# jizongFox/Deep-Co-Training-for-Semi-Supervised-Image-Segmentation

Hardware: AMD Instinct MI355X
Metric: co-train imgs/sec/node (lab+unlab), 2xUNet ACDC 256x256 (higher is better)
Workload: dtype bf16; 1 GPU; cfg2: 2xUNet co-training (CE + JSD), ACDC-shaped 256x256 C=4, bs 8+8 per GPU; global_batch=8+8, parallelism=dp1, inputs=blob-structured synthetic slices (tests/helpers.py::blob_batches)

## Files before the change

deep-co-training-for-semi-supervised-image-segmentation_amd/csrc/dct_common.h:

```cpp
#pragma once
#include <hip/hip_runtime.h>
#include <cstdio>
#include <stdint.h>
#include "../../include/dct.h"

typedef __bf16 bf16_t;
typedef __attribute__((ext_vector_type(8))) __bf16 bf16x8;
typedef __attribute__((ext_vector_type(4))) __bf16 bf16x4;
typedef __attribute__((ext_vector_type(2))) __bf16 bf16x2;
typedef _Float16 f16_t;
typedef __attribute__((ext_vector_type(8))) _Float16 f16x8;
typedef __attribute__((ext_vector_type(4))) _Float16 f16x4;
typedef __attribute__((ext_vector_type(16))) float f32x16;
typedef __attribute__((ext_vector_type(4))) float f32x4;
typedef __attribute__((ext_vector_type(2))) float f32x2;

#define DCT_WAVE 64

template <typename T> struct dct_type_of;
template <> struct dct_type_of<float> { static constexpr int id = DCT_F32; };
template <> struct dct_type_of<bf16_t> { static constexpr int id = DCT_BF16; };
template <> struct dct_type_of<f16_t> { static constexpr int id = DCT_F16; };

__device__ __forceinline__ float to_f32(float v) { return v; }
// ... 65 lines not shown
  *reinterpret_cast<dct_u32x2*>(p) = __builtin_bit_cast(dct_u32x2, v);
#endif
}

__device__ __forceinline__ unsigned dct_positive_bits8(dct_u32x4 w) {
  unsigned t[4];
#pragma unroll
  for (int k = 0; k < 4; ++k)
    asm("v_pk_max_i16 %0, %1, %2\n\tv_pk_min_u16 %0, %0, %3" : "=&v"(t[k]) : "v"(w[k]), "v"(0u), "v"(0x00010001u));
  const unsigned u = t[0] | (t[1] << 2) | (t[2] << 4) | (t[3] << 6);
  return u | (u >> 15);
}

void dct_prof_begin(int cls, hipStream_t s);
void dct_prof_end(int cls, hipStream_t s);
extern int g_dct_prof_on;

extern thread_local char g_dct_last_plan[200];
#define DCT_PLAN_NOTE(...) snprintf(g_dct_last_plan, sizeof(g_dct_last_plan), __VA_ARGS__)

extern int g_dct_skip_families;
enum { DCT_DIAG_IGEMM_SPLIT_MAX_TILES = 1002, DCT_DIAG_IGEMM_SPLIT_MIN_KITERS = 1003,
       DCT_DIAG_IGEMM_POOL = 1005,
       DCT_DIAG_STEM_DGRAD_MFMA = 1008,
       DCT_DIAG_SKIP_FAMILIES = 1100 };
enum { DCT_FAM_IGEMM2 = 1, DCT_FAM_IGEMM3M = 2, DCT_FAM_IGEMM3P = 4, DCT_FAM_WGRAD2 = 8, DCT_FAM_WGRAD3 = 16, DCT_FAM_FOLDS = 32,
       DCT_FAM_ADAM = 64, DCT_FAM_POINTWISE = 128 };
#define DCT_LAUNCH_FAM(fam, cls, kernel, grid, block, shmem, stream, ...)              \
  do {                                                                                 \
    if (g_dct_skip_families & (fam)) break;                                            \
    DCT_LAUNCH(cls, kernel, grid, block, shmem, stream, __VA_ARGS__);                  \
  } while (0)

#define DCT_LAUNCH(cls, kernel, grid, block, shmem, stream, ...)                       \
  do {                                                                                 \
    if (((cls) == DCT_PROF_POINTWISE && (g_dct_skip_families & 128)) || ((cls) == DCT_PROF_ADAM && (g_dct_skip_families & 64))) break; \
    if (g_dct_prof_on) dct_prof_begin((cls), (stream));                                \
    hipLaunchKernelGGL(kernel, grid, block, shmem, stream, __VA_ARGS__);               \
    if (g_dct_prof_on) dct_prof_end((cls), (stream));                                  \
  } while (0)

static inline int dct_check_launch() {
  return hipGetLastError() == hipSuccess ? DCT_OK : DCT_ERR_LAUNCH;
}

static inline unsigned div_up(long long a, long long b) { return (unsigned)((a + b - 1) / b); }
// ... 1 lines not shown
```

deep-co-training-for-semi-supervised-image-segmentation_amd/csrc/igemm.hip:

```cpp
#include <algorithm>
#include "igemm_common.h"

extern int g_tune_lean;

namespace {


template <typename T> struct Mfma;
template <> struct Mfma<bf16_t> {
  static constexpr int KSTEP = 16;
  __device__ static __forceinline__ void run(const char* a_row, const char* b_row, int half, f32x16& acc, int kk) {
    const bf16x8 a = *reinterpret_cast<const bf16x8*>(a_row + kk * 32 + half * 16);
    const bf16x8 b = *reinterpret_cast<const bf16x8*>(b_row + kk * 32 + half * 16);
    acc = __builtin_amdgcn_mfma_f32_32x32x16_bf16(a, b, acc, 0, 0, 0);
  }
};
template <> struct Mfma<float> {
  static constexpr int KSTEP = 2;
  __device__ static __forceinline__ void run(const char* a_row, const char* b_row, int half, f32x16& acc, int kk) {
    const float a = *reinterpret_cast<const float*>(a_row + (kk * 2 + half) * 4);
    const float b = *reinterpret_cast<const float*>(b_row + (kk * 2 + half) * 4);
    acc = __builtin_amdgcn_mfma_f32_32x32x2f32(a, b, acc, 0, 0, 0);
  }
};
// ... 456 lines not shown
      *reinterpret_cast<f32x4*>(slab + (long long)row * p.N + cc * 4) = v;
    }
    return;
  }
#pragma unroll
  for (int j = 0; j < TM; ++j) {
    const int m = m0 + wm * WTM + j * 32 + l31;
    if (m >= p.M) continue;
    const int hw = p.Ho * p.Wo;
    const int n = m / hw, rem = m - n * hw;
    const int oy = rem / p.Wo, ox = rem - oy * p.Wo;
#pragma unroll
    for (int i = 0; i < TN; ++i) {
#pragma unroll
      for (int q = 0; q < 4; ++q) {
        const int c = n0 + wn * WTN + i * 32 + 8 * q + 4 * half;
        float v[4] = {acc[i][j][4 * q + 0], acc[i][j][4 * q + 1], acc[i][j][4 * q + 2], acc[i][j][4 * q + 3]};
        epilogue_store4<bf16_t>(p, n, oy, ox, c, v);
      }
    }
  }
}

template <int BN, int NWM, int NWN, int ABUFS>
__global__ __launch_bounds__(NWM * NWN * 64) void igemm3m_kernel(IgemmParams p, int tiles_x, int tiles_y) {
  constexpr int NW = NWM * NWN;
  constexpr int TH = 8, TW = 16, BM = TH * TW, HW = TW + 2, HROWS = (TH + 2) * HW;
  constexpr int APIECES = (HROWS + 7) / 8, A_BYTES = APIECES * 8 * 128;
  constexpr int B_BYTES = BN * 128, BPIECES = BN / 8;
  constexpr int NPA = (APIECES + NW - 1) / NW, NPB = BPIECES / NW;
  constexpr int WTN = BN / NWN, TN = WTN / 32;
  static_assert(NWM == 4 && BPIECES % NW == 0 && TN >= 1, "tile/wave mismatch");
  constexpr int PXB = 8 / NWM;
  extern __shared__ __attribute__((aligned(128))) char smem[];
  char* Abuf = smem;
  char* Bbuf = smem + ABUFS * A_BYTES;

  const int tid = threadIdx.x, lane = tid & 63;
  const int wave = __builtin_amdgcn_readfirstlane(tid >> 6);
  const int wn = wave / NWM, wm = wave % NWM;
  int bx = blockIdx.x;
  const int ntile = blockIdx.y;
  const int tx = bx % tiles_x; bx /= tiles_x;
  const int ty = bx % tiles_y; const int img = bx / tiles_y;
  const int y0 = ty * TH, x0 = tx * TW, n0 = ntile * BN;
  const long long Ktot = 9ll * p.Cin;
  const bf16_t* xb = reinterpret_cast<const bf16_t*>(p.x);
  const char* zero = reinterpret_cast<const char*>(g_zero_page) + (lane & 7) * 16;

  int aoff[NPA];
#pragma unroll
  for (int i = 0; i < NPA; ++i) {
    const int piece = wave + i * NW;
    const int row = piece * 8 + (lane >> 3);
    aoff[i] = -1;
    if (piece < APIECES && row < HROWS) {
      const int hy = row / HW, hx = row - hy * HW;
      const int iy = y0 - p.pad_h + hy, ix = x0 - p.pad_w + hx;
      if ((unsigned)iy < (unsigned)p.Hi && (unsigned)ix < (unsigned)p.Wi)
        aoff[i] = (int)(img * p.xsN + iy * p.xsH + ix * p.xsW + (((lane & 7) ^ ((row >> 1) & 7)) * 8));
    }
  }
  auto stageA = [&](char* buf, int c0) {
#pragma unroll
    for (int i = 0; i < NPA; ++i) {
      const int piece = wave + i * NW;
      if (piece < APIECES) {
        const char* src = aoff[i] >= 0 ? reinterpret_cast<const char*>(xb + aoff[i] + c0) : zero;
        __builtin_amdgcn_global_load_lds((gptr_t)src, (lptr_t)(buf + piece * 1024), 16, 0, 0);
      }
    }
  };
  const bf16_t* wsrc[NPB];
#pragma unroll
  for (int i = 0; i < NPB; ++i) {
    const int row = (wave + i * NW) * 8 + (lane >> 3);
    wsrc[i] = reinterpret_cast<const bf16_t*>(p.w) + (long long)(n0 + row) * Ktot + (((lane & 7) ^ ((row >> 1) & 7)) * 8);
  }
  auto stageB = [&](char* buf, int tap, int c0) {
    const long long woff = (long long)tap * p.Cin + c0;
#pragma unroll
    for (int i = 0; i < NPB; ++i)
      __builtin_amdgcn_global_load_lds((gptr_t)(wsrc[i] + woff), (lptr_t)(buf + (wave + i * NW) * 1024), 16, 0, 0);
  };

  constexpr int TR = WTN / 16;
  f32x4 acc[TR][PXB];
#pragma unroll
  for (int i = 0; i < TR; ++i)
#pragma unroll
    for (int j = 0; j < PXB; ++j) acc[i][j] = f32x4{0.f, 0.f, 0.f, 0.f};

  const int l15 = lane & 15, kq = lane >> 4;
  const int rho0 = (PXB * wm) * HW + l15;
  const int aswz = (l15 >> 1) & 7;

  const int nch = p.Cin / 64;
  const unsigned smem_l = (unsigned)(size_t)(lptr_c)(smem);
  unsigned stem_gates[PXB] = {};
  float stem_xv = 0.f;
  if constexpr (BN == 64 && NWN == 1 && ABUFS == 1) {
    if (p.stem_x) {
#pragma unroll
      for (int j = 0; j < PXB; ++j) {
        const int oy = y0 + PXB * wm + j, ox = x0 + (lane & 15);
        if (oy < p.Ho && ox < p.Wo) {
// ... 7 lines not shown
        const int hy = tid / 18, hx = tid - hy * 18;
        const int iy = y0 + hy, ix = x0 + hx;
        if (iy < p.Ho + 2 && ix < p.Wo + 2) stem_xv = p.stem_x[((long long)img * (p.Ho + 2) + iy) * (p.Wo + 2) + ix];
      }
    }
  }
  stageA(Abuf, 0);
  stageB(Bbuf, 0, 0);
  float* biasL = reinterpret_cast<float*>(smem + ABUFS * A_BYTES + 2 * B_BYTES);
  if (tid < BN) biasL[tid] = p.bias ? p.bias[n0 + tid] : 0.f;
  __syncthreads();
  const unsigned Wb0 = smem_l + ABUFS * A_BYTES + (wn * WTN + l15) * 128 + ((kq ^ aswz) * 16);
  const bool wave_live = y0 + PXB * wm < p.Ho;
  int ab = 0, bb = 0;
  for (int c = 0; c < nch; ++c) {
    const unsigned Xs = smem_l + ab * A_BYTES;
#pragma unroll 1
    for (int t = 0; t < 9; ++t) {
      const int sx = t % 3, rr = t / 3;
      if (t < 8) stageB(Bbuf + (bb ^ 1) * B_BYTES, t + 1, c * 64);
      else if (c + 1 < nch) stageB(Bbuf + (bb ^ 1) * B_BYTES, 0, (c + 1) * 64);
      if (ABUFS == 2 && t == 0 && c + 1 < nch) stageA(Abuf + (ab ^ 1) * A_BYTES, (c + 1) * 64);
      if (wave_live) {
      const unsigned wa0 = Wb0 + bb * B_BYTES, wa1 = wa0 ^ 64u;
      unsigned rho_t = rho0;
      asm volatile("" : "+v"(rho_t));
      const unsigned pi0 = rho_t + rr * HW + sx;
      const unsigned xrow = Xs + (pi0 << 7);
      unsigned xj[PXB];
#pragma unroll
      for (int j = 0; j < PXB; ++j) xj[j] = xrow | (((kq ^ ((pi0 + j * HW) >> 1)) & 7) << 4);
      bf16x8 a[2][TR], b[2][PXB];
      RdRows<0, TR, 16 * 128>::run(wa0, a[0]);
      RdCols<0, PXB, HW * 128>::run(xj, 0u, b[0]);
      RdRows<0, TR, 16 * 128>::run(wa1, a[1]);
      RdCols<0, PXB, HW * 128>::run(xj, 64u, b[1]);
#pragma unroll
      for (int k2 = 0; k2 < 2; ++k2) {
        if (k2 == 0) lgkm_wait3<TR + PXB>(); else lgkm_wait3<0>();
#pragma unroll
        for (int i = 0; i < TR; ++i) touch8(a[k2][i]);
#pragma unroll
        for (int j = 0; j < PXB; ++j) touch8(b[k2][j]);
        __builtin_amdgcn_sched_barrier(0);
#pragma unroll
        for (int i = 0; i < TR; ++i)
#pragma unroll
          for (int j = 0; j < PXB; ++j)
            acc[i][j] = __builtin_amdgcn_mfma_f32_16x16x32_bf16(a[k2][i], b[k2][j], acc[i][j], 0, 0, 0);
      }
      }
      __syncthreads();
      bb ^= 1;
    }
    ab ^= 1;
  }

  constexpr int CPR = BN / 8;
  static_assert(BM * BN * 2 <= ABUFS * A_BYTES + (BN * 128 * 2 - BM * 8), "epilogue tile does not fit");
  char* tile = smem;
  if constexpr (BN == 64 && NWN == 1 && ABUFS == 1) {
    if (p.stem_x) {
      asm volatile("" ::: "memory");
      constexpr int XS = 32 * 1024, RED = 16 * 1024;
      unsigned short* xs = reinterpret_cast<unsigned short*>(smem + XS);
      if (tid < 180) {
        const bf16_t vh = (bf16_t)stem_xv;
        const bf16_t vl = (bf16_t)(stem_xv - (float)vh);
        xs[tid] = __builtin_bit_cast(unsigned short, vh);
        xs[180 + tid] = __builtin_bit_cast(unsigned short, vl);
      }
#pragma unroll
      for (int j = 0; j < PXB; ++j) {
        const int py = PXB * wm + j;
        const int row = py * TW + l15;
#pragma unroll
        for (int i = 0; i < TR; ++i) {
          const int cl = i * 16 + 4 * kq;
          const unsigned gate = (stem_gates[j] >> (8 * i + (cl & 4))) & 15u;
          bf16x4 o;
#pragma unroll
          for (int e = 0; e < 4; ++e) o[e] = (bf16_t)(((gate >> e) & 1u) ? acc[i][j][e] : 0.f);
// ... 26 lines not shown
        asm volatile("ds_read_b64_tr_b16 %0, %1" : "=v"(b1) : "v"(a1));
        asm volatile("s_waitcnt lgkmcnt(0)" ::: "memory");
        bf16x8 bb;
#pragma unroll
        for (int e = 0; e < 4; ++e) { bb[e] = b0[e]; bb[4 + e] = b1[e]; }
        touch8(bb);
        f32x4 z = {0.f, 0.f, 0.f, 0.f};
        z = __builtin_amdgcn_mfma_f32_16x16x32_bf16(al.v, bb, z, 0, 0, 0);
        sacc[nb] = __builtin_amdgcn_mfma_f32_16x16x32_bf16(ah.v, bb, z, 0, 0, 0);
      }
      float* red = reinterpret_cast<float*>(smem + RED);
#pragma unroll
      for (int nb = 0; nb < 4; ++nb) *reinterpret_cast<f32x4*>(red + ((wave * 4 + nb) * 64 + lane) * 4) = sacc[nb];
      __syncthreads();
      float* slab = p.stem_slab + (long long)blockIdx.x * 640;
      for (int idx = tid; idx < 640; idx += NW * 64) {
        const int ch = idx / 10, t = idx - ch * 10;
        const int o = ((ch >> 4) * 64 + (t >> 2) * 16 + (ch & 15)) * 4 + (t & 3);
        slab[idx] = (red[o] + red[o + 1024]) + (red[o + 2048] + red[o + 3072]);
      }
      return;
    }
  }
  int* rowY = reinterpret_cast<int*>(smem + ABUFS * A_BYTES + 2 * B_BYTES - BM * 8);
  int* rowM = rowY + BM;
  if (tid < BM) {
    const int oy = y0 + (tid >> 4), ox = x0 + (tid & 15);
    int oy_ = -1, om_ = -1;
    if (oy < p.Ho && ox < p.Wo) {
      oy_ = (int)(img * p.ysN + oy * p.ysH + ox * p.ysW);
      om_ = (int)(img * p.msN + oy * p.msH + ox * p.msW);
    }
    rowY[tid] = oy_; rowM[tid] = om_;
  }
  {
    f32x4 bv[TR];
#pragma unroll
    for (int i = 0; i < TR; ++i) bv[i] = *reinterpret_cast<const f32x4*>(biasL + wn * WTN + i * 16 + 4 * kq);
#pragma unroll
    for (int j = 0; j < PXB; ++j) {
      const int row = (PXB * wm + j) * TW + l15;
#pragma unroll
      for (int i = 0; i < TR; ++i) {
        const int cl = wn * WTN + i * 16 + 4 * kq;
        float v[4] = {acc[i][j][0] + bv[i][0], acc[i][j][1] + bv[i][1], acc[i][j][2] + bv[i][2], acc[i][j][3] + bv[i][3]};
        if (p.relu) {
#pragma unroll
          for (int e = 0; e < 4; ++e) v[e] = relu1(v[e]);
        }
        bf16x4 o;
#pragma unroll
        for (int e = 0; e < 4; ++e) o[e] = (bf16_t)v[e];
        const int chunk = (cl >> 3) ^ (row & (CPR - 1));
        *reinterpret_cast<bf16x4*>(tile + row * (BN * 2) + chunk * 16 + (cl & 4) * 2) = o;
      }
    }
  }
  __syncthreads();
  if (p.pool_y) {
    asm volatile("" ::: "memory");
    staged_pool_out<BN, NW>(p, tile, img, y0, x0, n0, tid);
    if (p.pool_only) return;
  }
  staged_rows_out<BM, BN, NW>(p, tile, rowY, rowM, n0, tid);
}

template <int BN, int NWM, int NWN, bool LEAN>
__global__ __launch_bounds__(NWM * NWN * 64) void igemm3p_kernel(IgemmParams p, int PR, int tiles_per_img, int chunks_per_split) {
  constexpr int NW = NWM * NWN;
  constexpr int BM = 128, APIECES = 24, A_BYTES = APIECES * 1024;
  constexpr int B_BYTES = BN * 128, BPIECES = BN / 8;
  constexpr int NPA = APIECES / NW, NPB = BPIECES / NW;
  constexpr int WTN = BN / NWN, TN = WTN / 32;
  static_assert(NWM == 4 && APIECES % NW == 0 && BPIECES % NW == 0 && TN >= 1, "tile/wave mismatch");
  extern __shared__ __attribute__((aligned(128))) char smem[];
  char* Abuf = smem;
  char* Bbuf = smem + 2 * A_BYTES;

  const int tid = threadIdx.x, lane = tid & 63;
  const int wave = __builtin_amdgcn_readfirstlane(tid >> 6);
  const int wn = wave / NWM, wm = wave % NWM;
  int bxi, byi, bzi;
  if (!xcd_remap(p, bxi, byi, bzi)) return;
  const int img = bxi / tiles_per_img, ty = bxi - img * tiles_per_img;
  const int y0 = ty * PR, n0 = byi * BN;
  const int pitch = p.Wo + 2, hrows = (PR + 2) * pitch;
  const long long Ktot = 9ll * p.Cin;
// ... 271 lines not shown
  }
}

__global__ __launch_bounds__(256) void relu_bits_kernel(const bf16_t* __restrict__ y, unsigned char* __restrict__ bits, long long chunks) {
  const long long i = (long long)blockIdx.x * 256 + threadIdx.x;
  if (i >= chunks) return;
  bits[i] = (unsigned char)relu_bits8(*reinterpret_cast<const bf16x8*>(y + 8 * i));
}

struct Plan {
  int bn, bm, splits, kiters, kiters_per_split, bk;
  int v2;
  int bounds;
  long long tiles;
};

int g_tune_igemm_split_target = 450;
int g_tune_igemm_split = -1;
int g_tune_igemm_split_max_tiles = 96;
int g_tune_igemm_split_min_kiters = 4;
int g_tune_igemm_halo_cover = 75;
int g_tune_igemm_halo_min_blocks = 400;
int g_tune_igemm_pool = 1;
int g_tune_igemm_halo = 1;

static bool tap_channels_ok(const dct_view* x, int N, int dtype) { return x->c % (dtype == DCT_BF16 ? 32 : 16) == 0 && N % 64 == 0; }
static bool make_plan(const dct_view* x, const dct_view* y, const dct_conv_desc* d, int dtype, int M, int N, Plan& pl) {
  if (!tap_channels_ok(x, N, dtype)) return false;
  pl.v2 = (dtype == DCT_BF16 && x->c % 64 == 0) ? 1 : 0;
  if (pl.v2) {
    pl.bk = 64;
    if (N % 128 == 0) { pl.bn = 128; pl.bm = 128; } else { pl.bn = 64; pl.bm = 256; }
    const int Ho = d->scatter2x2 ? y->h / 2 : y->h, Wo = d->scatter2x2 ? y->w / 2 : y->w;
    const bool inside = d->pad_h == 0 && d->pad_w == 0 &&
                        (Ho - 1) * d->stride + (d->R - 1) * d->dil < x->h &&
                        (Wo - 1) * d->stride + (d->S - 1) * d->dil < x->w;
    pl.bounds = inside ? 0 : 1;
  } else {
    pl.bk = dtype == DCT_BF16 ? 32 : 16;
    pl.bn = (N % 128 == 0) ? 128 : 64;
    pl.bm = 128;
    pl.bounds = 1;
  }
  pl.kiters = d->R * d->S * (x->c / pl.bk);
  pl.tiles = (long long)div_up(M, pl.bm) * (N / pl.bn);
  int splits = 1;
// ... 25 lines not shown
                              hipFuncAttributeMaxDynamicSharedMemorySize, (int)lds);
    attr_set = true;
  }
  DCT_LAUNCH_FAM(DCT_FAM_IGEMM2, DCT_PROF_IGEMM, (igemm2_kernel<BM, BN, WM, WN, BOUNDS, LEAN>), grid, dim3(WM * WN * 64), lds, st, p);
}
template <int BM, int BN, int WM, int WN, bool BOUNDS>
static void launch_v2(const IgemmParams& p, dim3 grid, hipStream_t st) {
  if ((g_tune_lean & 8) && p.x_bytes < (1ll << 31) && p.w_bytes < (1ll << 31) && p.R * p.S <= 32)
    launch_v2_k<BM, BN, WM, WN, BOUNDS, true>(p, grid, st);
  else launch_v2_k<BM, BN, WM, WN, BOUNDS, false>(p, grid, st);
}

template <int BN, int NWN, int ABUFS>
static void launch_v3(const IgemmParams& p, int tiles_x, int tiles_y, int images, hipStream_t st) {
  constexpr size_t lds = ABUFS * (size_t)(23 * 1024) + 2 * (size_t)BN * 128 + (size_t)BN * 4;
  static bool attr_set = false;
  if (!attr_set) {
    (void)hipFuncSetAttribute(reinterpret_cast<const void*>(&igemm3m_kernel<BN, 4, NWN, ABUFS>),
                              hipFuncAttributeMaxDynamicSharedMemorySize, (int)lds);
    attr_set = true;
  }
  const dim3 grid((unsigned)(images * tiles_y * tiles_x), p.N / BN, 1);
  DCT_LAUNCH_FAM(DCT_FAM_IGEMM3M, DCT_PROF_IGEMM, (igemm3m_kernel<BN, 4, NWN, ABUFS>), grid, dim3(4 * NWN * 64), lds, st, p, tiles_x, tiles_y);
}

struct PlanP { int use, PR, tiles_per_img, splits, cps; };
int g_tune_igemm_packed = 1;
int g_tune_igemm_packed_split = 160;
int g_tune_igemm_packed_fill = 50;
static PlanP make_plan_p(const dct_view* x, const dct_view* y, const dct_conv_desc* d, int dtype, int N) {
  PlanP pp = {0, 0, 0, 1, 0};
  if (!g_tune_igemm_halo || !g_tune_igemm_packed || dtype != DCT_BF16 || d->R != 3 || d->S != 3 || d->stride != 1 || d->dil != 1 ||
      d->scatter2x2 || x->c % 64 || N % 128 || y->w > 126)
    return pp;
  const int Wo = y->w, Ho = y->h;
  int PR = 128 / Wo;
  const int by_lds = 192 / (Wo + 2) - 2;
  if (PR > by_lds) PR = by_lds;
  if (PR > Ho) PR = Ho;
  if (PR < 1) return pp;
  const int tiles = (Ho + PR - 1) / PR;
  if ((double)Ho * Wo / (tiles * 128.0) < g_tune_igemm_packed_fill * 0.01) return pp;
  const int nch = x->c / 64;
  const long long blocks0 = (long long)y->n * tiles * (N / 128);
  int splits = 1;
  if (blocks0 < g_tune_igemm_packed_split) {
// ... 54 lines not shown
  } else if (pl.bn == 128) {
    DCT_LAUNCH(DCT_PROF_IGEMM, (igemm_kernel<T, 128, 128>), grid, dim3(256), 0, st, p);
  } else {
    DCT_LAUNCH(DCT_PROF_IGEMM, (igemm_kernel<T, 64, 128>), grid, dim3(256), 0, st, p);
  }
  fold_splits<T>(p, pl.splits, st);
}

}

void dct_split_dw_db_launch(const float* partial, float* scratch, float* dw, float* db, int cout, int inner, int blocks, int accumulate, hipStream_t st);
size_t dct_split_dw_db_scratch(int cout, int inner);

void dct_relu_bits_launch(const void* y_bf16, unsigned char* bits, long long chunks, hipStream_t st) {
  DCT_LAUNCH(DCT_PROF_POINTWISE, relu_bits_kernel, dim3(div_up(chunks, 256)), dim3(256), 0, st, (const bf16_t*)y_bf16, bits, chunks);
}

enum Route { ROUTE_HALO, ROUTE_HALO_STEM, ROUTE_PACKED, ROUTE_TAP };
struct ConvPlan {
  Route route;
  Plan tap;
  PlanP packed;
  int bn, tiles_x, tiles_y; long long blocks; double cover;
  int staged;
  int fused_pool;
  int bits_after;
  size_t workspace;
};
struct ConvPtrs { bool vec16; size_t workspace_bytes; };
static bool vec16_ok(const dct_view* v, int channels) {
  return !((uintptr_t)v->ptr & 15) && v->sw % 8 == 0 && v->sh % 8 == 0 && v->sn % 8 == 0 && channels % 8 == 0 && (long long)v->n * v->sn < (1ll << 31);
}
static bool bias16_ok(const float* bias) { return !bias || !((uintptr_t)bias & 15); }
static size_t slab_bytes(int splits, int M, int N) { return splits > 1 ? (size_t)splits * M * N * sizeof(float) : 0; }

static int plan_conv(const dct_view* x, const dct_view* y, const dct_conv_desc* d, int dtype, const ConvPtrs* ptrs, ConvPlan& cp) {
  const int Ho = d->scatter2x2 ? y->h / 2 : y->h, Wo = d->scatter2x2 ? y->w / 2 : y->w;
  const int M = y->n * Ho * Wo, N = d->scatter2x2 ? 4 * y->c : y->c;
  const Plan& pl = cp.tap;
  if (!make_plan(x, y, d, dtype, M, N, cp.tap)) return DCT_ERR_UNSUPPORTED;
  const size_t tap_need = slab_bytes(pl.splits, M, N);
  cp.tiles_y = (Ho + 7) / 8; cp.tiles_x = (Wo + 15) / 16; cp.bn = N % 128 == 0 ? 128 : 64;
  const long long patches = (long long)y->n * cp.tiles_y * cp.tiles_x;
  cp.blocks = patches * (N / cp.bn);
  cp.cover = (double)Ho * Wo / ((double)cp.tiles_y * 8 * cp.tiles_x * 16);
  const bool x32 = (long long)x->n * x->sn < (1ll << 31) && (long long)cp.bn * 9 * x->c * 2 < (1ll << 32);
  const bool halo = pl.v2 && pl.splits == 1 && g_tune_igemm_halo && d->R == 3 && d->S == 3 && d->stride == 1 && d->dil == 1 && !d->scatter2x2 &&
                    x32 && cp.cover >= g_tune_igemm_halo_cover * 0.01 && cp.blocks >= g_tune_igemm_halo_min_blocks && (cp.bn == 128 || x->c == 64);
  const size_t stem_need = d->stem_x ? (size_t)patches * 640 * sizeof(float) + dct_split_dw_db_scratch(64, 9) : 0;
  cp.packed = make_plan_p(x, y, d, dtype, N);
  const size_t packed_need = cp.packed.use ? slab_bytes(cp.packed.splits, M, N) : 0;
  cp.staged = cp.fused_pool = cp.bits_after = 0;
  if (!ptrs) { cp.workspace = std::max({tap_need, packed_need, stem_need}); return DCT_OK; }
  if (ptrs->workspace_bytes < tap_need) return DCT_ERR_WORKSPACE;
  cp.staged = (pl.v2 && pl.splits == 1 && !d->accumulate && ptrs->vec16) ? 1 : 0;
  if (halo && ptrs->vec16) {
    cp.route = d->stem_x ? ROUTE_HALO_STEM : ROUTE_HALO;
    cp.fused_pool = (d->pool_out && g_tune_igemm_pool) ? 1 : 0;
    cp.workspace = stem_need;
    return ptrs->workspace_bytes < stem_need ? DCT_ERR_WORKSPACE : DCT_OK;
  }
  if (d->stem_x) return DCT_ERR_UNSUPPORTED;
  if (cp.packed.use && ptrs->vec16 && ptrs->workspace_bytes >= packed_need) {
    cp.route = ROUTE_PACKED; cp.workspace = packed_need;
    return DCT_OK;
  }
  cp.route = ROUTE_TAP; cp.workspace = tap_need;
  cp.bits_after = (d->relu_bits_out && !cp.staged && pl.splits == 1) ? 1 : 0;
  return DCT_OK;
}

// ... 60 lines not shown
  }
  const ConvPtrs ptrs = {vec16_ok(y, y->c) && (!mask || vec16_ok(mask, p.mask_channels)) && bias16_ok(bias), workspace ? workspace_bytes : 0};
  ConvPlan cp;
  const int rc = plan_conv(x, y, d, dtype, &ptrs, cp);
  if (rc != DCT_OK) return rc;
  p.relu = d->relu; p.accumulate = d->accumulate;
  p.kiters = cp.tap.kiters; p.kiters_per_split = cp.tap.kiters_per_split;
  p.cin_iters = x->c / cp.tap.bk;
  p.staged = cp.staged;
  p.x_bytes = view_span(x) * esz;
  p.w_bytes = (long long)p.N * d->R * d->S * x->c * esz;
  p.xcd_gx = p.xcd_gy = 1;
  p.Hp = (y->h + 1) / 2; p.Wp = (y->w + 1) / 2;
  hipStream_t st = (hipStream_t)stream;
  switch (cp.route) {
    case ROUTE_HALO_STEM:
      p.stem_x = d->stem_x; p.stem_slab = (float*)workspace;
      launch_v3<64, 1, 1>(p, cp.tiles_x, cp.tiles_y, y->n, st);
      dct_split_dw_db_launch(p.stem_slab, p.stem_slab + cp.blocks * 640, d->stem_dw, d->stem_db, 64, 9, (int)cp.blocks, d->stem_accumulate, st);
      DCT_PLAN_NOTE("igemm3m shared-halo 8x16 patches x 64 ch: %lld blocks, stem weight gradient from the tile, y not stored", cp.blocks);
      break;
    case ROUTE_HALO:
      if (cp.fused_pool) { p.pool_y = (char*)d->pool_out; p.pool_codes = d->pool_codes; p.pool_only = d->pool_only ? 1 : 0; }
      if (cp.bn == 128) {
        if (x->c == 64) launch_v3<128, 2, 1>(p, cp.tiles_x, cp.tiles_y, y->n, st); else launch_v3<128, 2, 2>(p, cp.tiles_x, cp.tiles_y, y->n, st);
      } else launch_v3<64, 1, 1>(p, cp.tiles_x, cp.tiles_y, y->n, st);
      DCT_PLAN_NOTE("igemm3m shared-halo 8x16 patches x %d ch: %lld blocks, cover %.0f %%, %d K-steps%s", cp.bn, cp.blocks, cp.cover * 100, 9 * x->c / 64,
                    p.pool_y ? (p.pool_only ? ", pooled in the epilogue, y not stored" : ", pooled in the epilogue") : "");
      break;
    case ROUTE_PACKED:
      if (cp.packed.splits > 1) p.partial = (float*)workspace;
      launch_v3p(p, cp.packed, y->n, st);
      DCT_PLAN_NOTE("igemm3p packed rows (%d rows of %d px per 128-px tile): %d x %d blocks x %d channel-slice splits", cp.packed.PR, p.Wo,
                    y->n * cp.packed.tiles_per_img, p.N / 128, cp.packed.splits);
      break;
    case ROUTE_TAP:
      if (cp.tap.splits > 1) p.partial = (float*)workspace;
      if (dtype == DCT_BF16) launch<bf16_t>(p, cp.tap, st); else launch<float>(p, cp.tap, st);
      DCT_PLAN_NOTE("%s per-tap %d x %d tile%s: %lld tiles x %d splits, %d K-steps each%s", cp.tap.v2 ? "igemm2" : "igemm", cp.tap.bm, cp.tap.bn,
                    cp.tap.bounds ? " (bounds)" : "", cp.tap.tiles, cp.tap.splits, cp.tap.kiters_per_split, p.staged ? ", staged epilogue" : "");
      break;
  }
  if (cp.bits_after) dct_relu_bits_launch(y->ptr, p.bits_out, (long long)y->n * y->h * y->w * (y->c / 8), st);
  if (d->pool_out && !cp.fused_pool) {
    dct_view pv;
    pv.ptr = d->pool_out; pv.n = y->n; pv.h = p.Hp; pv.w = p.Wp; pv.c = y->c;
    pv.sw = y->c; pv.sh = (long long)p.Wp * y->c; pv.sn = (long long)p.Hp * p.Wp * y->c;
    const int rp = d->pool_codes ? dct_maxpool2x2_fwd_codes(y, &pv, d->pool_codes, dtype, stream) : dct_maxpool2x2_fwd(y, &pv, dtype, stream);
    if (rp != DCT_OK) return rp;
  }
  return dct_check_launch();
}


int dct_tune_set_wgrad(int knob, int value);
extern int g_enet_wgrad_max_blocks;
extern int g_enet_mfma;
extern int g_stem_dgrad_mfma;
extern int g_enet_mwgrad_waves;

extern "C" int dct_tune_set(int knob, int value) {
  switch (knob) {
    case DCT_TUNE_IGEMM_SPLIT: g_tune_igemm_split = value; return DCT_OK;
    case DCT_TUNE_IGEMM_HALO: g_tune_igemm_halo = value; return DCT_OK;
    case DCT_TUNE_IGEMM_PACKED: g_tune_igemm_packed = value; return DCT_OK;
    case DCT_TUNE_IGEMM_HALO_MIN_BLOCKS: g_tune_igemm_halo_min_blocks = value; return DCT_OK;
    case DCT_TUNE_IGEMM_HALO_COVER: g_tune_igemm_halo_cover = value; return DCT_OK;
    case DCT_TUNE_IGEMM_SPLIT_TARGET: if (value < 64) return DCT_ERR_BAD_ARG; g_tune_igemm_split_target = value; return DCT_OK;
    case DCT_TUNE_ENET_MWGRAD_WAVES: if (value < 64) return DCT_ERR_BAD_ARG; g_enet_mwgrad_waves = value; return DCT_OK;
    case DCT_TUNE_ENET_MFMA: if (value < 0 || value > 3) return DCT_ERR_BAD_ARG; g_enet_mfma = value; return DCT_OK;
    case DCT_TUNE_IGEMM_PACKED_SPLIT: if (value < 1) return DCT_ERR_BAD_ARG; g_tune_igemm_packed_split = value; return DCT_OK;
    case DCT_TUNE_IGEMM_PACKED_FILL: if (value < 1 || value > 100) return DCT_ERR_BAD_ARG; g_tune_igemm_packed_fill = value; return DCT_OK;
    case DCT_TUNE_IGEMM_XCD: if (value < 0 || value > 2) return DCT_ERR_BAD_ARG; g_tune_igemm_xcd = value; return DCT_OK;
    case DCT_DIAG_SKIP_FAMILIES: g_dct_skip_families = value; return DCT_OK;
    case DCT_DIAG_IGEMM_POOL: g_tune_igemm_pool = value ? 1 : 0; return DCT_OK;
    case DCT_DIAG_STEM_DGRAD_MFMA: g_stem_dgrad_mfma = value ? 1 : 0; return DCT_OK;
    case DCT_DIAG_IGEMM_SPLIT_MAX_TILES: g_tune_igemm_split_max_tiles = value; return DCT_OK;
    case DCT_DIAG_IGEMM_SPLIT_MIN_KITERS: g_tune_igemm_split_min_kiters = value; return DCT_OK;
    case DCT_TUNE_ENET_WGRAD_BLOCKS: if (value < 1 || value > 1024) return DCT_ERR_BAD_ARG; g_enet_wgrad_max_blocks = value; return DCT_OK;
    default: return dct_tune_set_wgrad(knob, value);
  }
}
```

deep-co-training-for-semi-supervised-image-segmentation_amd/csrc/igemm_common.h:

```cpp
#pragma once
#include "dct_common.h"

namespace {

struct IgemmParams {
  const char* x; const char* w; const float* bias; const char* mask; char* y;
  const unsigned char* mask_bits;
  unsigned char* bits_out;
  float* partial;
  int M, N, Cin, R, S;
  int Ho, Wo, Hi, Wi;
  int stride, dil, pad_h, pad_w;
  long long xsN, xsH, xsW;
  long long ysN, ysH, ysW;
  long long msN, msH, msW;
  int relu, scatter, accumulate, mask_channels;
  float mask_scale;
  int kiters, kiters_per_split, cin_iters;
  int cout;
  int staged;
  long long x_bytes, w_bytes;
  char* pool_y;
  unsigned char* pool_codes;
  int Hp, Wp;
// ... 66 lines not shown
      if (p.mask_bits) mb[t] = p.mask_bits[(unsigned)(rowM[row] + co) >> 3];
      else if (p.mask && co < p.mask_channels) mk[t] = *reinterpret_cast<const bf16x8*>(reinterpret_cast<const bf16_t*>(p.mask) + rowM[row] + co);
      if (p.accumulate) old[t] = *reinterpret_cast<const bf16x8*>(reinterpret_cast<const bf16_t*>(p.y) + yo[t] + co);
    }
  }
#pragma unroll
  for (int t = 0; t < NCH; ++t) {
    const int id = t * (NW * 64) + tid;
    const int row = id / CPR, cc = id % CPR;
    if (yo[t] < 0) continue;
    bf16x8 v = *reinterpret_cast<const bf16x8*>(tile + row * (BN * 2) + ((cc ^ (row & (CPR - 1))) * 16));
    const int co = n0 + cc * 8;
    if (p.mask_bits) chunk_gate_bits(v, mb[t], p.mask_scale);
    else if (p.mask && co < p.mask_channels) chunk_gate_act(v, mk[t], p.mask_scale);
    if (p.accumulate) {
      asm volatile("" ::: "memory");
      chunk_add(v, old[t]);
    }
    dct_store16_stream(reinterpret_cast<bf16_t*>(p.y) + yo[t] + co, v);
    if (p.bits_out) p.bits_out[(unsigned)(yo[t] + co) >> 3] = (unsigned char)relu_bits8(v);
  }
}

template <int BN, int NW>
__device__ __forceinline__ void staged_pool_out(const IgemmParams& p, const char* tile, int img, int y0, int x0, int n0, int tid) {
  constexpr int CPR = BN / 8;
  for (int id = tid; id < 32 * CPR; id += NW * 64) {
    const int cc = id % CPR, q = id / CPR;
    const int qy = q >> 3, qx = q & 7;
    const int oy = y0 + 2 * qy, ox = x0 + 2 * qx;
    if (oy >= p.Ho || ox >= p.Wo) continue;
    float m[8];
    int arg[8];
#pragma unroll
    for (int i = 0; i < 8; ++i) { m[i] = -INFINITY; arg[i] = 8; }
#pragma unroll
    for (int k = 0; k < 4; ++k) {
      if (oy + (k >> 1) < p.Ho && ox + (k & 1) < p.Wo) {
        const int row = (2 * qy + (k >> 1)) * 16 + 2 * qx + (k & 1);
        const bf16x8 v = *reinterpret_cast<const bf16x8*>(tile + row * (BN * 2) + ((cc ^ (row & (CPR - 1))) * 16));
#pragma unroll
        for (int i = 0; i < 8; ++i) {
          const float f = (float)v[i];
          if (f > m[i]) { m[i] = f; arg[i] = k; }
        }
      }
    }
    const long long o = (((long long)img * p.Hp + (oy >> 1)) * p.Wp + (ox >> 1)) * p.cout + n0 + cc * 8;
    bf16x8 out;
#pragma unroll
// ... 14 lines not shown
  const int logical = (L & 7) * per + (L >> 3);
  if (logical >= p.xcd_total) return false;
  bx = logical % p.xcd_gx;
  const int rest = logical / p.xcd_gx;
  by = rest % p.xcd_gy; bz = rest / p.xcd_gy;
  return true;
}

__device__ __forceinline__ float relu1(float v) {
  float r;
  asm("v_max_f32 %0, 0, %1" : "=v"(r) : "v"(v));
  return r;
}

__device__ __attribute__((aligned(128))) const uint4 g_zero_page[8] = {};

typedef __attribute__((address_space(1))) const void* gptr_t;
typedef __attribute__((address_space(3))) void* lptr_t;
typedef __attribute__((address_space(3))) const char* lptr_c;
__device__ __forceinline__ void rd128(unsigned addr, bf16x8& dst) { asm volatile("ds_read_b128 %0, %1" : "=v"(dst) : "v"(addr)); }
template <int OFF> __device__ __forceinline__ void rd128o(unsigned addr, bf16x8& dst) {
  asm volatile("ds_read_b128 %0, %1 offset:%2" : "=v"(dst) : "v"(addr), "n"(OFF));
}
template <int I, int N, int STRIDE> struct RdRows {
  __device__ static __forceinline__ void run(unsigned addr, bf16x8 (&dst)[N]) {
    rd128o<I * STRIDE>(addr, dst[I]);
    if constexpr (I + 1 < N) RdRows<I + 1, N, STRIDE>::run(addr, dst);
  }
};
template <int J, int N, int STRIDE> struct RdCols {
  __device__ static __forceinline__ void run(const unsigned (&addr)[N], unsigned flip, bf16x8 (&dst)[N]) {
    rd128o<J * STRIDE>(addr[J] ^ flip, dst[J]);
    if constexpr (J + 1 < N) RdCols<J + 1, N, STRIDE>::run(addr, flip, dst);
  }
};
__device__ __forceinline__ void buf_lds16(__amdgpu_buffer_rsrc_t r, unsigned lds, int voff, unsigned soff) {
  __builtin_amdgcn_raw_ptr_buffer_load_lds(r, (lptr_t)(size_t)lds, 16, voff, (int)soff, 0, 0);
}
#define DCT_BUF_INVALID ((int)0x80000000u)
template <int N> __device__ __forceinline__ void lgkm_wait3() { asm volatile("s_waitcnt lgkmcnt(%0)" ::"n"(N) : "memory"); }
__device__ __forceinline__ void touch8(bf16x8& r) { asm volatile("" : "+v"(r)); }

}
```

include/dct.h:

```cpp
#ifndef DCT_H_
#define DCT_H_

#include <stddef.h>
#include <stdint.h>

#ifdef __cplusplus
extern "C" {
#endif

typedef enum dct_status {
  DCT_OK = 0,
  DCT_ERR_BAD_ARG = -1,
  DCT_ERR_UNSUPPORTED = -2,
  DCT_ERR_LAUNCH = -3,
  DCT_ERR_WORKSPACE = -4
} dct_status;

typedef enum dct_dtype { DCT_F32 = 0, DCT_BF16 = 1, DCT_F16 = 2 } dct_dtype;

typedef struct dct_view {
  void* ptr;
  int32_t n, h, w, c;
  int64_t sn, sh, sw;
} dct_view;
// ... 246 lines not shown
int dct_confusion_counts(const float* const* logits, int S, const int64_t* gt ,
                         int B, int64_t pixels_per_image, int C, int32_t* counts , dct_stream stream);

enum { DCT_PROF_IGEMM = 0, DCT_PROF_WGRAD = 1, DCT_PROF_POINTWISE = 2, DCT_PROF_LOSS = 3,
       DCT_PROF_ADAM = 4, DCT_PROF_OTHER = 5, DCT_PROF_NCLASS = 6 };
int dct_prof_enable(int on);
enum { DCT_TUNE_IGEMM_SPLIT = 1,
       DCT_TUNE_WGRAD_CHUNKS = 3,
       DCT_TUNE_IGEMM_HALO = 7,
       DCT_TUNE_WGRAD_ROWS = 8,
       DCT_TUNE_WGRAD_ROWS_FILL = 9,
       DCT_TUNE_IGEMM_PACKED = 10,
       DCT_TUNE_ENET_WGRAD_BLOCKS = 12,
       DCT_TUNE_WGRAD_TARGET = 14,
       DCT_TUNE_WGRAD3_TARGET = 15,
       DCT_TUNE_IGEMM_SPLIT_TARGET = 16,
       DCT_TUNE_IGEMM_HALO_MIN_BLOCKS = 19,
       DCT_TUNE_IGEMM_HALO_COVER = 20,
       DCT_TUNE_IGEMM_PACKED_SPLIT = 23,
       DCT_TUNE_IGEMM_PACKED_FILL = 24,
       DCT_TUNE_ENET_MFMA = 26,
       DCT_TUNE_ENET_MWGRAD_WAVES = 28,
       DCT_TUNE_IGEMM_XCD = 39,
       DCT_TUNE_LEAN = 38 };
int dct_tune_set(int knob, int value);
int dct_prof_read(double* ms_per_class, int64_t* launches_per_class, int reset);
int dct_clock_probe(unsigned long long* out2, unsigned long long ref_ticks, dct_stream stream);
int dct_stamp(unsigned long long* slot, unsigned ring, dct_stream stream);

typedef struct dct_enet_bwd_in {
  const dct_view* g; const dct_view* g_mask;
  const float* mean; const float* invstd; const float* c1c2;
} dct_enet_bwd_in;
int dct_enet_conv_bwd_in(const dct_view* raw, const float* w, const dct_enet_tf* tf, const dct_enet_bwd_in* bin,
                         const dct_view* y, const dct_conv_desc* d, int transposed, int ws_out, int ws_tap, int ws_in,
                         const dct_view* resid_grad, const dct_view* resid_mask, int f32_mask, int dtype,
                         const dct_view* bn_raw, const float* bn_scale, const float* bn_shift, const float* bn_slope, int bn_act,
                         const float* bn_mean, const float* bn_invstd,
                         double* stats_partial, int stats_capacity_rows, int* stats_rows, dct_stream stream);
int dct_enet_bn_bwd_sums(const dct_view* raw, const dct_view* g, const dct_view* g_mask,
                         const float* scale, const float* shift, const float* slope, int act,
                         const float* mean, const float* invstd,
                         float* dgamma, float* dbeta, float* dslope, float* c1c2, int training,
                         int f32_mask, int dtype, void* workspace, size_t workspace_bytes, int partial_rows, dct_stream stream);
int dct_enet_bn_bwd_apply(const dct_view* raw, const dct_view* g, const dct_view* g_mask,
                          const float* scale, const float* shift, const float* slope, int act,
// ... 17 lines not shown
```

Baseline: 4825 imgs/sec.

## Add tall 16x16-patch shared-halo igemm variant with software-pipelined LDS reads

Adds a TH=16 variant of the shared-halo 3x3 implicit-GEMM kernel. It covers 16x16 output patches per block, so each halo load is amortised over twice as many rows. The new kernel uses a single halo buffer, double-buffered LDS reads interleaved with MFMAs under explicit waitcnts, and a fixed 4-waves-per-EU occupancy. The planner picks it for BN=128 convolutions when coverage and block count pass thresholds. The cost is fewer blocks, a serialised restage of A between channel chunks, and a tight LDS budget for the epilogue.

```diff
diff --git a/deep-co-training-for-semi-supervised-image-segmentation_amd/csrc/dct_common.h b/deep-co-training-for-semi-supervised-image-segmentation_amd/csrc/dct_common.h
--- a/deep-co-training-for-semi-supervised-image-segmentation_amd/csrc/dct_common.h
+++ b/deep-co-training-for-semi-supervised-image-segmentation_amd/csrc/dct_common.h
@@ -111,6 +111,7 @@
 extern int g_dct_skip_families;
 enum { DCT_DIAG_IGEMM_SPLIT_MAX_TILES = 1002, DCT_DIAG_IGEMM_SPLIT_MIN_KITERS = 1003,
        DCT_DIAG_IGEMM_POOL = 1005,
+       DCT_DIAG_IGEMM_HALO_TALL_MIN_BLOCKS = 1009,
        DCT_DIAG_STEM_DGRAD_MFMA = 1008,
        DCT_DIAG_SKIP_FAMILIES = 1100 };
 enum { DCT_FAM_IGEMM2 = 1, DCT_FAM_IGEMM3M = 2, DCT_FAM_IGEMM3P = 4, DCT_FAM_WGRAD2 = 8, DCT_FAM_WGRAD3 = 16, DCT_FAM_FOLDS = 32,
diff --git a/deep-co-training-for-semi-supervised-image-segmentation_amd/csrc/igemm.hip b/deep-co-training-for-semi-supervised-image-segmentation_amd/csrc/igemm.hip
--- a/deep-co-training-for-semi-supervised-image-segmentation_amd/csrc/igemm.hip
+++ b/deep-co-training-for-semi-supervised-image-segmentation_amd/csrc/igemm.hip
@@ -502,16 +502,82 @@
   }
 }
 
-template <int BN, int NWM, int NWN, int ABUFS>
-__global__ __launch_bounds__(NWM * NWN * 64) void igemm3m_kernel(IgemmParams p, int tiles_x, int tiles_y) {
+__device__ __forceinline__ void lgkm_wait_n(int n) {
+  switch (n) {
+    case 0: lgkm_wait3<0>(); break;
+    case 1: lgkm_wait3<1>(); break;
+    case 2: lgkm_wait3<2>(); break;
+    case 3: lgkm_wait3<3>(); break;
+    case 4: lgkm_wait3<4>(); break;
+    case 5: lgkm_wait3<5>(); break;
+    case 6: lgkm_wait3<6>(); break;
+    default: lgkm_wait3<7>(); break;
+  }
+}
+template <int TR, int PXB, int HW>
+__device__ __forceinline__ void tall_tap(unsigned wa0, unsigned Xs, unsigned rho0, int tap_rows, int kq, f32x4 (&acc)[TR][PXB]) {
+  static_assert(TR <= 4 && PXB <= 4, "immediate offsets and wait counts");
+  const unsigned wa1 = wa0 ^ 64u;
+  unsigned rho_t = rho0;
+  asm volatile("" : "+v"(rho_t));
+  const unsigned pi0 = rho_t + tap_rows;
+  const unsigned xrow = Xs + (pi0 << 7);
+  unsigned xj[PXB];
+#pragma unroll
+  for (int j = 0; j < PXB; ++j) xj[j] = xrow | (((kq ^ ((pi0 + j * HW) >> 1)) & 7) << 4);
+  bf16x8 a[TR], b[PXB];
+  RdRows<0, TR, 16 * 128>::run(wa0, a);
+  RdCols<0, PXB, HW * 128>::run(xj, 0u, b);
+#pragma unroll
+  for (int j = 0; j < PXB; ++j) {
+    lgkm_wait_n(PXB - 1);
+    if (j == 0) {
+#pragma unroll
+      for (int i = 0; i < TR; ++i) touch8(a[i]);
+    }
+    touch8(b[j]);
+    __builtin_amdgcn_sched_barrier(0);
+#pragma unroll
+    for (int i = 0; i < TR; ++i) {
+      acc[i][j] = __builtin_amdgcn_mfma_f32_16x16x32_bf16(a[i], b[j], acc[i][j], 0, 0, 0);
+      if (j == PXB - 1) {
+        __builtin_amdgcn_sched_barrier(0);
+        rd128o_dyn(wa1, i * 16 * 128, a[i]);
+      }
+    }
+    __builtin_amdgcn_sched_barrier(0);
+    rd128o_dyn(xj[j] ^ 64u, j * HW * 128, b[j]);
+  }
+#pragma unroll
+  for (int i = 0; i < TR; ++i) {
+    lgkm_wait_n(TR - i);
+    touch8(a[i]);
+    if (i == 0) {
+#pragma unroll
+      for (int j = 0; j < PXB - 1; ++j) touch8(b[j]);
+    }
+    __builtin_amdgcn_sched_barrier(0);
+#pragma unroll
+    for (int j = 0; j < PXB - 1; ++j) acc[i][j] = __builtin_amdgcn_mfma_f32_16x16x32_bf16(a[i], b[j], acc[i][j], 0, 0, 0);
+    __builtin_amdgcn_sched_barrier(0);
+  }
+  lgkm_wait_n(0);
+  touch8(b[PXB - 1]);
+  __builtin_amdgcn_sched_barrier(0);
+#pragma unroll
+  for (int i = 0; i < TR; ++i) acc[i][PXB - 1] = __builtin_amdgcn_mfma_f32_16x16x32_bf16(a[i], b[PXB - 1], acc[i][PXB - 1], 0, 0, 0);
+}
+
+template <int BN, int NWM, int NWN, int ABUFS, int TH>
+__device__ __forceinline__ void igemm3m_body(const IgemmParams& p, int tiles_x, int tiles_y) {
   constexpr int NW = NWM * NWN;
-  constexpr int TH = 8, TW = 16, BM = TH * TW, HW = TW + 2, HROWS = (TH + 2) * HW;
+  constexpr int TW = 16, BM = TH * TW, HW = TW + 2, HROWS = (TH + 2) * HW;
   constexpr int APIECES = (HROWS + 7) / 8, A_BYTES = APIECES * 8 * 128;
   constexpr int B_BYTES = BN * 128, BPIECES = BN / 8;
   constexpr int NPA = (APIECES + NW - 1) / NW, NPB = BPIECES / NW;
   constexpr int WTN = BN / NWN, TN = WTN / 32;
-  static_assert(NWM == 4 && BPIECES % NW == 0 && TN >= 1, "tile/wave mismatch");
-  constexpr int PXB = 8 / NWM;
+  static_assert(NWM == 4 && BPIECES % NW == 0 && TN >= 1 && (TH == 8 || (TH == 16 && ABUFS == 1)), "tile/wave mismatch");
+  constexpr int PXB = TH / NWM;
   extern __shared__ __attribute__((aligned(128))) char smem[];
   char* Abuf = smem;
   char* Bbuf = smem + ABUFS * A_BYTES;
@@ -546,7 +612,9 @@
     for (int i = 0; i < NPA; ++i) {
       const int piece = wave + i * NW;
       if (piece < APIECES) {
-        const char* src = aoff[i] >= 0 ? reinterpret_cast<const char*>(xb + aoff[i] + c0) : zero;
+        int ao = aoff[i];
+        if constexpr (TH == 16) asm volatile("" : "+v"(ao));
+        const char* src = ao >= 0 ? reinterpret_cast<const char*>(xb + ao + c0) : zero;
         __builtin_amdgcn_global_load_lds((gptr_t)src, (lptr_t)(buf + piece * 1024), 16, 0, 0);
       }
     }
@@ -560,8 +628,10 @@
   auto stageB = [&](char* buf, int tap, int c0) {
     const long long woff = (long long)tap * p.Cin + c0;
 #pragma unroll
-    for (int i = 0; i < NPB; ++i)
-      __builtin_amdgcn_global_load_lds((gptr_t)(wsrc[i] + woff), (lptr_t)(buf + (wave + i * NW) * 1024), 16, 0, 0);
+    for (int i = 0; i < NPB; ++i) {
+      const bf16_t* src = TH == 16 ? wsrc[0] + (woff + (long long)i * (NW * 8) * Ktot) : wsrc[i] + woff;
+      __builtin_amdgcn_global_load_lds((gptr_t)src, (lptr_t)(buf + (wave + i * NW) * 1024), 16, 0, 0);
+    }
   };
 
   constexpr int TR = WTN / 16;
@@ -615,6 +685,9 @@
       else if (c + 1 < nch) stageB(Bbuf + (bb ^ 1) * B_BYTES, 0, (c + 1) * 64);
       if (ABUFS == 2 && t == 0 && c + 1 < nch) stageA(Abuf + (ab ^ 1) * A_BYTES, (c + 1) * 64);
       if (wave_live) {
+      if constexpr (TH == 16) {
+        tall_tap<TR, PXB, HW>(Wb0 + bb * B_BYTES, Xs, rho0, rr * HW + sx, kq, acc);
+      } else {
       const unsigned wa0 = Wb0 + bb * B_BYTES, wa1 = wa0 ^ 64u;
       unsigned rho_t = rho0;
       asm volatile("" : "+v"(rho_t));
@@ -643,14 +716,20 @@
             acc[i][j] = __builtin_amdgcn_mfma_f32_16x16x32_bf16(a[k2][i], b[k2][j], acc[i][j], 0, 0, 0);
       }
       }
+      }
       __syncthreads();
       bb ^= 1;
     }
-    ab ^= 1;
+    if constexpr (ABUFS == 2) ab ^= 1;
+    if constexpr (TH == 16) if (c + 1 < nch) {
+      stageA(Abuf, (c + 1) * 64);
+      __syncthreads();
+    }
   }
 
   constexpr int CPR = BN / 8;
-  static_assert(BM * BN * 2 <= ABUFS * A_BYTES + (BN * 128 * 2 - BM * 8), "epilogue tile does not fit");
+  static_assert(BM * BN * 2 <= ABUFS * A_BYTES + (BN * 128 * 2 - BM * 8),
+                "epilogue tile does not fit (TH = 16, BN = 128: 64 KiB in 41 KiB of halo stage + 32 KiB of weight stages - 2 KiB of row tables)");
   char* tile = smem;
   if constexpr (BN == 64 && NWN == 1 && ABUFS == 1) {
     if (p.stem_x) {
@@ -723,16 +802,17 @@
       return;
     }
   }
+  const int tid_e = TH == 16 ? wave * 64 + (int)__builtin_amdgcn_mbcnt_hi(~0u, __builtin_amdgcn_mbcnt_lo(~0u, 0u)) : tid;
   int* rowY = reinterpret_cast<int*>(smem + ABUFS * A_BYTES + 2 * B_BYTES - BM * 8);
   int* rowM = rowY + BM;
-  if (tid < BM) {
-    const int oy = y0 + (tid >> 4), ox = x0 + (tid & 15);
+  if (tid_e < BM) {
+    const int oy = y0 + (tid_e >> 4), ox = x0 + (tid_e & 15);
     int oy_ = -1, om_ = -1;
     if (oy < p.Ho && ox < p.Wo) {
       oy_ = (int)(img * p.ysN + oy * p.ysH + ox * p.ysW);
       om_ = (int)(img * p.msN + oy * p.msH + ox * p.msW);
     }
-    rowY[tid] = oy_; rowM[tid] = om_;
+    rowY[tid_e] = oy_; rowM[tid_e] = om_;
   }
   {
     f32x4 bv[TR];
@@ -760,10 +840,18 @@
   __syncthreads();
   if (p.pool_y) {
     asm volatile("" ::: "memory");
-    staged_pool_out<BN, NW>(p, tile, img, y0, x0, n0, tid);
+    staged_pool_out<BN, NW, TH>(p, tile, img, y0, x0, n0, tid_e);
     if (p.pool_only) return;
   }
-  staged_rows_out<BM, BN, NW>(p, tile, rowY, rowM, n0, tid);
+  staged_rows_out<BM, BN, NW>(p, tile, rowY, rowM, n0, tid_e);
+}
+template <int BN, int NWM, int NWN, int ABUFS>
+__global__ __launch_bounds__(NWM * NWN * 64) void igemm3m_kernel(IgemmParams p, int tiles_x, int tiles_y) {
+  igemm3m_body<BN, NWM, NWN, ABUFS, 8>(p, tiles_x, tiles_y);
+}
+template <int BN, int NWM, int NWN>
+__global__ __launch_bounds__(NWM * NWN * 64) __attribute__((amdgpu_waves_per_eu(4, 4))) void igemm3m_tall_kernel(IgemmParams p, int tiles_x, int tiles_y) {
+  igemm3m_body<BN, NWM, NWN, 1, 16>(p, tiles_x, tiles_y);
 }
 
 template <int BN, int NWM, int NWN, bool LEAN>
@@ -1081,6 +1169,8 @@
 int g_tune_igemm_halo_cover = 75;
 int g_tune_igemm_halo_min_blocks = 400;
 int g_tune_igemm_pool = 1;
+int g_tune_igemm_halo_tall = 1;
+int g_tune_igemm_halo_tall_min_blocks = 512;
 int g_tune_igemm_halo = 1;
 
 static bool tap_channels_ok(const dct_view* x, int N, int dtype) { return x->c % (dtype == DCT_BF16 ? 32 : 16) == 0 && N % 64 == 0; }
@@ -1152,6 +1242,19 @@
   }
   const dim3 grid((unsigned)(images * tiles_y * tiles_x), p.N / BN, 1);
   DCT_LAUNCH_FAM(DCT_FAM_IGEMM3M, DCT_PROF_IGEMM, (igemm3m_kernel<BN, 4, NWN, ABUFS>), grid, dim3(4 * NWN * 64), lds, st, p, tiles_x, tiles_y);
+}
+
+template <int BN, int NWN>
+static void launch_v3_tall(const IgemmParams& p, int tiles_x, int tiles_y, int images, hipStream_t st) {
+  constexpr size_t lds = (size_t)(41 * 1024) + 2 * (size_t)BN * 128 + (size_t)BN * 4;
+  static bool attr_set = false;
+  if (!attr_set) {
+    (void)hipFuncSetAttribute(reinterpret_cast<const void*>(&igemm3m_tall_kernel<BN, 4, NWN>),
+                              hipFuncAttributeMaxDynamicSharedMemorySize, (int)lds);
+    attr_set = true;
+  }
+  const dim3 grid((unsigned)(images * tiles_y * tiles_x), p.N / BN, 1);
+  DCT_LAUNCH_FAM(DCT_FAM_IGEMM3M, DCT_PROF_IGEMM, (igemm3m_tall_kernel<BN, 4, NWN>), grid, dim3(4 * NWN * 64), lds, st, p, tiles_x, tiles_y);
 }
 
 struct PlanP { int use, PR, tiles_per_img, splits, cps; };
@@ -1252,6 +1355,7 @@
   Plan tap;
   PlanP packed;
   int bn, tiles_x, tiles_y; long long blocks; double cover;
+  int th;
   int staged;
   int fused_pool;
   int bits_after;
@@ -1275,8 +1379,17 @@
   cp.blocks = patches * (N / cp.bn);
   cp.cover = (double)Ho * Wo / ((double)cp.tiles_y * 8 * cp.tiles_x * 16);
   const bool x32 = (long long)x->n * x->sn < (1ll << 31) && (long long)cp.bn * 9 * x->c * 2 < (1ll << 32);
-  const bool halo = pl.v2 && pl.splits == 1 && g_tune_igemm_halo && d->R == 3 && d->S == 3 && d->stride == 1 && d->dil == 1 && !d->scatter2x2 &&
-                    x32 && cp.cover >= g_tune_igemm_halo_cover * 0.01 && cp.blocks >= g_tune_igemm_halo_min_blocks && (cp.bn == 128 || x->c == 64);
+  const bool halo_form = pl.v2 && pl.splits == 1 && g_tune_igemm_halo && d->R == 3 && d->S == 3 && d->stride == 1 && d->dil == 1 && !d->scatter2x2 && x32;
+  bool halo = halo_form && cp.cover >= g_tune_igemm_halo_cover * 0.01 && cp.blocks >= g_tune_igemm_halo_min_blocks && (cp.bn == 128 || x->c == 64);
+  cp.th = 8;
+  if (g_tune_igemm_halo_tall && halo_form && !d->stem_x && cp.bn == 128 && (halo || g_tune_igemm_halo_tall == 2)) {
+    const int ty16 = (Ho + 15) / 16;
+    const long long blocks16 = (long long)y->n * ty16 * cp.tiles_x * (N / 128);
+    const double cover16 = (double)Ho * Wo / ((double)ty16 * 16 * cp.tiles_x * 16);
+    if (g_tune_igemm_halo_tall == 2 || (cover16 >= g_tune_igemm_halo_cover * 0.01 && blocks16 >= g_tune_igemm_halo_tall_min_blocks)) {
+      cp.th = 16; cp.tiles_y = ty16; cp.blocks = blocks16; cp.cover = cover16; halo = true;
+    }
+  }
   const size_t stem_need = d->stem_x ? (size_t)patches * 640 * sizeof(float) + dct_split_dw_db_scratch(64, 9) : 0;
   cp.packed = make_plan_p(x, y, d, dtype, N);
   const size_t packed_need = cp.packed.use ? slab_bytes(cp.packed.splits, M, N) : 0;
@@ -1383,10 +1496,12 @@
       break;
     case ROUTE_HALO:
       if (cp.fused_pool) { p.pool_y = (char*)d->pool_out; p.pool_codes = d->pool_codes; p.pool_only = d->pool_only ? 1 : 0; }
-      if (cp.bn == 128) {
+      if (cp.th == 16) {
+        launch_v3_tall<128, 2>(p, cp.tiles_x, cp.tiles_y, y->n, st);
+      } else if (cp.bn == 128) {
         if (x->c == 64) launch_v3<128, 2, 1>(p, cp.tiles_x, cp.tiles_y, y->n, st); else launch_v3<128, 2, 2>(p, cp.tiles_x, cp.tiles_y, y->n, st);
       } else launch_v3<64, 1, 1>(p, cp.tiles_x, cp.tiles_y, y->n, st);
-      DCT_PLAN_NOTE("igemm3m shared-halo 8x16 patches x %d ch: %lld blocks, cover %.0f %%, %d K-steps%s", cp.bn, cp.blocks, cp.cover * 100, 9 * x->c / 64,
+      DCT_PLAN_NOTE("igemm3m shared-halo %dx16 patches x %d ch: %lld blocks, cover %.0f %%, %d K-steps%s", cp.th, cp.bn, cp.blocks, cp.cover * 100, 9 * x->c / 64,
                     p.pool_y ? (p.pool_only ? ", pooled in the epilogue, y not stored" : ", pooled in the epilogue") : "");
       break;
     case ROUTE_PACKED:
@@ -1427,6 +1542,8 @@
     case DCT_TUNE_IGEMM_PACKED: g_tune_igemm_packed = value; return DCT_OK;
     case DCT_TUNE_IGEMM_HALO_MIN_BLOCKS: g_tune_igemm_halo_min_blocks = value; return DCT_OK;
     case DCT_TUNE_IGEMM_HALO_COVER: g_tune_igemm_halo_cover = value; return DCT_OK;
+    case DCT_TUNE_IGEMM_HALO_TALL: if (value < 0 || value > 2) return DCT_ERR_BAD_ARG; g_tune_igemm_halo_tall = value; return DCT_OK;
+    case DCT_DIAG_IGEMM_HALO_TALL_MIN_BLOCKS: if (value < 1) return DCT_ERR_BAD_ARG; g_tune_igemm_halo_tall_min_blocks = value; return DCT_OK;
     case DCT_TUNE_IGEMM_SPLIT_TARGET: if (value < 64) return DCT_ERR_BAD_ARG; g_tune_igemm_split_target = value; return DCT_OK;
     case DCT_TUNE_ENET_MWGRAD_WAVES: if (value < 64) return DCT_ERR_BAD_ARG; g_enet_mwgrad_waves = value; return DCT_OK;
     case DCT_TUNE_ENET_MFMA: if (value < 0 || value > 3) return DCT_ERR_BAD_ARG; g_enet_mfma = value; return DCT_OK;
diff --git a/deep-co-training-for-semi-supervised-image-segmentation_amd/csrc/igemm_common.h b/deep-co-training-for-semi-supervised-image-segmentation_amd/csrc/igemm_common.h
--- a/deep-co-training-for-semi-supervised-image-segmentation_amd/csrc/igemm_common.h
+++ b/deep-co-training-for-semi-supervised-image-segmentation_amd/csrc/igemm_common.h
@@ -112,10 +112,10 @@
   }
 }
 
-template <int BN, int NW>
+template <int BN, int NW, int TH = 8>
 __device__ __forceinline__ void staged_pool_out(const IgemmParams& p, const char* tile, int img, int y0, int x0, int n0, int tid) {
   constexpr int CPR = BN / 8;
-  for (int id = tid; id < 32 * CPR; id += NW * 64) {
+  for (int id = tid; id < TH * 4 * CPR; id += NW * 64) {
     const int cc = id % CPR, q = id / CPR;
     const int qy = q >> 3, qx = q & 7;
     const int oy = y0 + 2 * qy, ox = x0 + 2 * qx;
@@ -176,6 +176,9 @@
 template <int OFF> __device__ __forceinline__ void rd128o(unsigned addr, bf16x8& dst) {
   asm volatile("ds_read_b128 %0, %1 offset:%2" : "=v"(dst) : "v"(addr), "n"(OFF));
 }
+__device__ __forceinline__ void rd128o_dyn(unsigned addr, int off, bf16x8& dst) {
+  asm volatile("ds_read_b128 %0, %1 offset:%2" : "=v"(dst) : "v"(addr), "i"(off));
+}
 template <int I, int N, int STRIDE> struct RdRows {
   __device__ static __forceinline__ void run(unsigned addr, bf16x8 (&dst)[N]) {
     rd128o<I * STRIDE>(addr, dst[I]);
diff --git a/include/dct.h b/include/dct.h
--- a/include/dct.h
+++ b/include/dct.h
@@ -292,6 +292,7 @@
        DCT_TUNE_ENET_MFMA = 26,
        DCT_TUNE_ENET_MWGRAD_WAVES = 28,
        DCT_TUNE_IGEMM_XCD = 39,
+       DCT_TUNE_IGEMM_HALO_TALL = 40,
        DCT_TUNE_LEAN = 38 };
 int dct_tune_set(int knob, int value);
 int dct_prof_read(double* ms_per_class, int64_t* launches_per_class, int reset);
```

After: 4957 imgs/sec, median of 6. +2.7%, better.
